# DSL-Lab/echoglad

Hardware: AMD Instinct MI355X
Metric: echo frames/sec through full GNN stack (224x224 default hier-graph); MAE parity (higher is better)
Workload: dtype f32; 1 GPU; configs[1] default.yml: 224x224 frame, 7 aux levels, num_gnn_layers=3, batch=8 per GPU, eval mode, node features [B*N,128] in HBM -> logits [B*N_valid,4] in HBM; workload_short=configs[1] default.yml: 224x224, 7 aux levels, L=3, batch 8/GPU, eval, nodes_per_frame=72020, directed_edges_per_frame=430200, global_batch=8, parallelism=dp1 (batch-sharded frames, no data-path collective), launch=hipGraph replay of the step's kernels

## Files before the change

echoglad_amd/build.py:

```python
from __future__ import annotations

import os
import shutil
import subprocess
import sys
from pathlib import Path

PKG = Path(__file__).resolve().parent
CSRC = PKG / "csrc"
LIBDIR = PKG / "lib"
LIBNAME = "libechoglad_hip.so"
SOURCES = ["graph.hip", "topo_tables.hip", "gcn_layer.hip", "gcn_layer_ps.hip", "conn.hip", "classifier.hip", "train.hip", "bn_act_tiles.hip", "cls_train.hip", "coord.hip", "coord_mlp.hip", "heatmap.hip", "pack.hip", "pool.hip", "adam.hip", "metrics.hip", "labels.hip", "frame_prep.hip", "frontend.hip", "frontend_train.hip", "embedder.hip"]
ARCH = "gfx950"


def hipcc() -> str:
    for cand in (os.environ.get("HIPCC"), shutil.which("hipcc"), "/opt/rocm/bin/hipcc"):
        if cand and os.path.exists(cand):
            return cand
    raise RuntimeError("hipcc not found; the HIP extension cannot be built")


def lib_path() -> Path:
    return LIBDIR / LIBNAME


def _stale(target: Path, deps) -> bool:
    if not target.exists():
        return True
    t = target.stat().st_mtime
    return any(Path(d).stat().st_mtime > t for d in deps)


def build(force: bool = False, verbose: bool = False, extra_flags=(), variant: str = "") -> Path:
    LIBDIR.mkdir(exist_ok=True)
    objdir = LIBDIR / ("obj" + ("_" + variant if variant else ""))
    objdir.mkdir(exist_ok=True)
    headers = list(CSRC.glob("*.h")) + [PKG.parent / "include" / "echoglad_hip.h"]
    cc = hipcc()
    flags = [f"--offload-arch={ARCH}", "-O3", "-fPIC", "-std=c++17", "-Wall", "-Wno-unused-function",
             "-mllvm", "-amdgpu-atomic-optimizer-strategy=None", *extra_flags]
    if verbose:
        flags.append("-Rpass-analysis=kernel-resource-usage")
    objs = []
    procs = []
    for src in SOURCES:
        s = CSRC / src
        if not s.exists():
            continue
        o = objdir / (s.stem + ".o")
        objs.append(o)
        if force or _stale(o, [s] + headers):
            cmd = [cc, *flags, "-c", str(s), "-o", str(o)]
            if verbose:
                print(" ".join(cmd), flush=True)
            procs.append((src, subprocess.Popen(cmd, stdout=subprocess.PIPE, stderr=subprocess.STDOUT, text=True)))
    for src, p in procs:
        out, _ = p.communicate()
        if verbose or p.returncode != 0:
            print(out, flush=True)
        if p.returncode != 0:
            raise RuntimeError(f"hipcc failed on {src}")
    target = lib_path() if not variant else LIBDIR / f"libechoglad_hip.{variant}.so"
    if force or _stale(target, objs):
        cmd = [cc, f"--offload-arch={ARCH}", "-shared", "-fPIC", "-o", str(target), *map(str, objs)]
        if verbose:
            print(" ".join(cmd), flush=True)
        subprocess.run(cmd, check=True)
    return target


if __name__ == "__main__":
    extra = [a for a in sys.argv[1:] if a.startswith("-D")]
    if "--" in sys.argv:
        extra += sys.argv[sys.argv.index("--") + 1:]
    var = [a.split("=", 1)[1] for a in sys.argv[1:] if a.startswith("--variant=")]
    p = build(force="--force" in sys.argv, verbose="--verbose" in sys.argv, extra_flags=extra,
              variant=var[0] if var else "")
    print(p)
```

echoglad_amd/csrc/common.h:

```cpp
#pragma once
#include <hip/hip_runtime.h>
#include <stdint.h>
#include <atomic>
#include <mutex>
#include <string>
#include <vector>

#include "../../include/echoglad_hip.h"

namespace eg {

constexpr int C = EG_CHANNELS;
constexpr int TILE = 64;
constexpr int LDA = C + 4;
constexpr int MAX_LEVELS = 14;
constexpr int MAX_SLOTS = 10;

int set_error(int code, const std::string& msg);
#define EG_HIP_TRY(expr)                                                                         \
    do {                                                                                         \
        hipError_t _e = (expr);                                                                  \
        if (_e != hipSuccess)                                                                    \
            return ::eg::set_error(EG_ERR_HIP, std::string(#expr) + ": " + hipGetErrorString(_e)); \
    } while (0)
// ... 75 lines not shown
    int r, c;
    if (is_main) {
        r = (int)(((unsigned long long)(unsigned)idx * T.magic) >> 40);
        c = idx - r * side;
    } else {
        const int lg = l + 1;
        r = idx >> lg;
        c = idx & (side - 1);
    }
    int deg = 0;
    nb.valid[1] = r > 0;            nb.id[1] = nb.valid[1] ? n - side : n;
    nb.valid[2] = r < side - 1;     nb.id[2] = nb.valid[2] ? n + side : n;
    nb.valid[3] = c > 0;            nb.id[3] = nb.valid[3] ? n - 1 : n;
    nb.valid[4] = c < side - 1;     nb.id[4] = nb.valid[4] ? n + 1 : n;
    deg += nb.valid[1] + nb.valid[2] + nb.valid[3] + nb.valid[4];
    if (is_main) {
        if (T.n_aux > 0 && r < 2 * T.ncrop && c < 2 * T.ncrop) {
            const int pl = T.n_levels - 2;
            nb.id[5] = T.base[pl] + (T.crop0 + (r >> 1)) * T.side[pl] + T.crop0 + (c >> 1);
            nb.valid[5] = 1; ++deg;
        }
        nb.count = 6;
    } else {
        if (l > 0) {
            nb.id[5] = T.base[l - 1] + (r >> 1) * T.side[l - 1] + (c >> 1);
            nb.valid[5] = 1; ++deg;
        }
        const int cl = l + 1;
        int cr = -1, cc = -1;
        if (cl < T.n_levels - 1) { cr = 2 * r; cc = 2 * c; }
        else if (r >= T.crop0 && r < T.crop0 + T.ncrop && c >= T.crop0 && c < T.crop0 + T.ncrop) {
            cr = 2 * (r - T.crop0); cc = 2 * (c - T.crop0);
        }
        if (cr >= 0) {
            const int cs = T.side[cl];
            const int b = T.base[cl] + cr * cs + cc;
            nb.id[6] = b;          nb.id[7] = b + 1;
            nb.id[8] = b + cs;     nb.id[9] = b + cs + 1;
            nb.valid[6] = nb.valid[7] = nb.valid[8] = nb.valid[9] = 1;
            deg += 4;
        }
        nb.count = 10;
    }
    nb.degree = deg;
}

enum GraphKind { GRAPH_TOPO = 1, GRAPH_CSR = 2 };

struct Knobs {
    int walk_mode;
    int stagger;
    int grid_cap;
    int layer_impl;
    int ps_grid;
    int ring_guard;
    int csr_tiles;
    int queue_self_reset;
};
Knobs read_knobs();
const Knobs& process_knobs();

constexpr int QUEUE_SLICE_INTS = 8 * 32;
constexpr int QUEUE_DONE_IDX = 1;
#ifdef EG_STAMP
constexpr int QUEUE_SLOTS = 1;
#else
constexpr int QUEUE_SLOTS = 64;
#endif
constexpr int QUEUE_TAIL_INTS = 64;
constexpr int EG_ERR_RING = -100;
inline int public_rc(int rc) { return rc == EG_ERR_RING ? EG_ERR_UNSUPPORTED : rc; }

}

struct eg_graph {
    int kind;
    int64_t n_nodes;
    eg::Topo topo;
    eg::Topo* topo_dev;
    eg::TileDesc* tiles_dev;
    eg::SegDesc* segs_dev;
    float* pats_dev;
    float* patsq_dev;
    int n_pats;
    int kid_rows;
    int hybrid;
    int n_conn;
    int conn_chunks;
    int* conn_table;
    mutable float* conn_scratch;
    mutable int conn_cap;
    mutable std::mutex conn_mutex;
    mutable std::vector<float*> conn_retired;
    int flat;
    int n_tiles;
    float* dis;
    int* rowptr;
    int* colidx;
    int64_t nnz;
    int* t_rows;
    int* t_rowptr;
    int* t_code;
    int* t_tgt;
    float* t_w;
    float* t_dis;
    int n_ctiles;
// ... 63 lines not shown
```

echoglad_amd/csrc/gcn_layer_ps.hip:

```cpp
#include <stdlib.h>

#include "seg_wide.h"
#include "train_common.h"

namespace eg {

constexpr int PS_THREADS = 512;
constexpr int PS_LDS_DIS = 4 * TILE * LDA + 16 + 64;
constexpr int PS_LDS_PAT = PS_LDS_DIS + 2 * TILE;

struct PsDims {
    int n_per_frame, batch, tiles_per_frame, relu, transpose_w, has_res;
    int kid_rows;
    int n_pats;
    float* agg_out;
    float* stats_partial;
    int static_walk;
    const float* res;
    const float* conn;
    int conn_stride, conn_agg, conn_scaled, n_conn;
    int self_reset;
    LowerSums lower;
};

// ... 22 lines not shown
#ifndef EG_PROBE_N
#define EG_PROBE_N 64
#endif
#define EG_PROBE(site) do { if ((site) == EG_PROBE_SITE) { int pa_ = lane, pb_ = lane; _Pragma("unroll") for (int i_ = 0; i_ < EG_PROBE_N / 2; ++i_) { \
    asm volatile("v_mov_b32 %0, %0" : "+v"(pa_)); asm volatile("v_mov_b32 %0, %0" : "+v"(pb_)); } asm volatile("" :: "v"(pa_), "v"(pb_)); } } while (0)
#else
#define EG_PROBE(site) do {} while (0)
#endif

__device__ inline int frame_of(int tile, int tiles_per_frame, int& hint) {
#ifdef EG_FRAME_HINT
    const unsigned t_in = (unsigned)(tile - hint * tiles_per_frame);
    if (t_in >= (unsigned)tiles_per_frame) hint = tile / tiles_per_frame;
    return hint;
#else
    (void)hint;
    return tile / tiles_per_frame;
#endif
}

__device__ inline float max_raw(float x, float y) {
    float r;
    asm("v_max_f32 %0, %1, %2" : "=v"(r) : "v"(x), "v"(y));
    return r;
}

__device__ inline int ps_claim_issue(int* __restrict__ counters, int group) {
    return atomicAdd(&counters[group * WALK_CTR_STRIDE], 1);
}
__device__ inline void ps_claim(int* __restrict__ counters, int group, int n_tiles, int* slot);
__device__ inline void ps_claim_commit(int* __restrict__ counters, int group, int n_tiles, int got, int* slot) {
    const int chunk = (n_tiles + WALK_GROUPS - 1) / WALK_GROUPS;
    const int lo = group * chunk;
    const int size = (n_tiles - lo) < chunk ? (n_tiles - lo) : chunk;
    if (got < size) *slot = lo + got;
    else ps_claim(counters, (group + 1) % WALK_GROUPS, n_tiles, slot);
}

__device__ inline void ps_claim(int* __restrict__ counters, int group, int n_tiles, int* slot) {
    const int chunk = (n_tiles + WALK_GROUPS - 1) / WALK_GROUPS;
    int t = -1;
    for (int k = 0; k < WALK_GROUPS && t < 0; ++k) {
        const int q = (group + k) % WALK_GROUPS;
        const int lo = q * chunk;
        const int size = (n_tiles - lo) < chunk ? (n_tiles - lo) : chunk;
        if (size <= 0) continue;
        const int got = atomicAdd(&counters[q * WALK_CTR_STRIDE], 1);
        if (got < size) t = lo + got;
    }
    *slot = t;
}


template <bool CLS, bool JK = false, int MODE = 0, bool DIAG = false, int FOLD = 0>
__global__ __launch_bounds__(PS_THREADS, 2) void k_gcn_layer_ps(const float* __restrict__ x, const float* __restrict__ W,
                                                                const float* __restrict__ scale, const float* __restrict__ shift,
                                                                float* __restrict__ out, const float* __restrict__ dis,
                                                                const Topo* __restrict__ T, const TileDesc* __restrict__ tiles,
                                                                const SegDesc* __restrict__ segs, const float* __restrict__ pats,
                                                                const float* __restrict__ patsq, const float* __restrict__ kin, float* __restrict__ kout,
                                                                const float* __restrict__ jk_in, float* __restrict__ jk_out,
                                                                int* __restrict__ counters, const PsDims a, const ClsArgs ca,
                                                                const int* __restrict__ rowptr, const int* __restrict__ colidx) {
    constexpr bool TRAIN = MODE == 1;
    constexpr bool RSEP = MODE >= 2;
    constexpr bool SUMS = MODE == 3;
    extern __shared__ __attribute__((aligned(16))) float smem[];
    float* s_a0 = smem;
    float* s_x0 = smem + 2 * TILE * LDA;
    int* s_tile = reinterpret_cast<int*>(smem + 4 * TILE * LDA);
    int* s_sync = s_tile + 8;
    int* s_cd = s_tile + 16;
    float* s_dis0 = smem + PS_LDS_DIS;
    float* s_pat = smem + PS_LDS_PAT;
    float* s_bn = s_pat + a.n_pats * PATQ;

    const int tid = threadIdx.x;
    const int lane_k = tid & 63;
    const int wave = wave_id();
    const bool consumer = wave < 4;
    const int n_tiles = a.tiles_per_frame * a.batch;
    const int group = xcc_id();

    if (tid == 256) {
        if (TRAIN && a.static_walk) {
            for (int i = 0; i < 3; ++i) s_tile[i] = ps_static_tile(i, n_tiles);
        } else {
            ps_claim(counters, group, n_tiles, &s_tile[0]);
            ps_claim(counters, group, n_tiles, &s_tile[1]);
            ps_claim(counters, group, n_tiles, &s_tile[2]);
        }
    }
    for (int i = tid; i < a.n_pats * PATQ; i += PS_THREADS) s_pat[i] = patsq[i];
    if (TRAIN) {
        for (int i = tid; i < 4 * TILE * LDA; i += PS_THREADS) smem[i] = 0.f;
    }
    static_assert(!FOLD || (CLS && !JK && MODE == 0), "FOLD is a form of the fused last layer without the running maximum");
    if (CLS) {
        if (FOLD) {
            if (tid < C) s_bn[tid] = ca.t1[tid];
        } else if (tid < C) {
            s_bn[tid] = scale ? scale[tid] : 1.0f;
            s_bn[C + tid] = shift ? shift[tid] : 0.0f;
            s_bn[2 * C + tid] = ca.s1[tid];
            s_bn[3 * C + tid] = ca.t1[tid];
        }
        if (tid == 0) *s_sync = 0;
    }
    __syncthreads();

    if (wave < 4) {
        constexpr bool RES_LATE = CLS;
        float wreg[64];
        load_w_slice(W, wave, lane_k, a.transpose_w, wreg);
        if (!FOLD && scale) {
            const float sv = scale[32 * wave + (lane_k & 31)];
#pragma unroll
            for (int t = 0; t < 64; ++t) wreg[t] *= sv;
        }
        f32x16 shv;
        if (!CLS) {
#pragma unroll
            for (int g = 0; g < 4; ++g) {
                const int ch0 = 32 * wave + 8 * g + 4 * (lane_k >> 5);
                const f32x4 q = shift ? *reinterpret_cast<const f32x4*>(shift + ch0) : f32x4{0.f, 0.f, 0.f, 0.f};
                shv[4 * g] = q.x; shv[4 * g + 1] = q.y; shv[4 * g + 2] = q.z; shv[4 * g + 3] = q.w;
            }
        }
        float wreg2[64];
        float w2a[8];
        f32x4 t2v, w3v;
        float b3v = 0.f;
        if (CLS) {
            load_w_slice(ca.w1, wave, lane_k, 0, wreg2);
            if (!FOLD) {
                const float sv = ca.s1[32 * wave + (lane_k & 31)];
#pragma unroll
                for (int t = 0; t < 64; ++t) wreg2[t] *= sv;
            }
            const f32x4* pw = reinterpret_cast<const f32x4*>(ca.w2 + (size_t)(wave * 16 + (lane_k & 15)) * 32 + 8 * (lane_k >> 4));
            const f32x4 q0 = pw[0], q1 = pw[1];
            w2a[0] = q0.x; w2a[1] = q0.y; w2a[2] = q0.z; w2a[3] = q0.w; w2a[4] = q1.x; w2a[5] = q1.y; w2a[6] = q1.z; w2a[7] = q1.w;
            {
                const float sv = ca.s2[wave * 16 + (lane_k & 15)];
#pragma unroll
                for (int t = 0; t < 8; ++t) w2a[t] *= sv;
            }
            const int o4 = wave * 16 + 4 * (lane_k >> 4);
            t2v = *reinterpret_cast<const f32x4*>(ca.t2 + o4);
            w3v = *reinterpret_cast<const f32x4*>(ca.w3 + o4);
            b3v = ca.b3[wave];
        }
        f32x16 csum, csq;
#pragma unroll
        for (int i = 0; i < 16; ++i) { csum[i] = 0.f; csq[i] = 0.f; }
        f32x4 lsc = {0.f, 0.f, 0.f, 0.f}, lsh = lsc;
        unsigned long long lseed = 0;
        if (SUMS) {
            lsc = *reinterpret_cast<const f32x4*>(a.lower.scale + 32 * wave + 4 * (lane_k & 7));
            lsh = *reinterpret_cast<const f32x4*>(a.lower.shift + 32 * wave + 4 * (lane_k & 7));
            lseed = a.lower.seed + epoch_now(a.lower.epoch);
        }
        __syncthreads();
        int frame_hint = 0;
        PSTAMP_INIT;
#ifdef EG_STAMP
        const unsigned long long clk0 = __builtin_amdgcn_s_memtime(), rt0 = __builtin_amdgcn_s_memrealtime();
#endif
        for (int k = 0;; ++k) {
            const int t_cur = __builtin_amdgcn_readfirstlane(s_tile[k & 7]);
            if (t_cur < 0) break;
            int lane = lane_k;
// ... 137 lines not shown
            auto read_segments = [&](int i0) {
#pragma unroll
                for (int e = 0; e < 4; ++e) {
                    if (JK) {
                        const int i = seg_cnt[i0 + e] > 0 ? i0 + e : 0;
                        const int cnt = seg_cnt[i0 + e] > 0 ? seg_cnt[i0 + e] : seg_cnt[0];
                        const int first = seg_cnt[i0 + e] > 0 ? seg_first[i0 + e] : seg_first[0];
                        const int u = u8 < cnt ? u8 : cnt - 1;
                        o[e] = *reinterpret_cast<const f32x4*>(s_x + (8 * i + u) * LDA + 32 * wave + c4);
                        node[e] = first + u;
                        ovoff[e] = u * (C * 4) + ocol;
                        osoff[e] = first * (C * 4);
                        jm[e] = *reinterpret_cast<const f32x4*>(jb + (size_t)node[e] * C);
                    } else {
                        const int last = seg_cnt[i0 + e] - 1;
                        const int u = u8 < last ? u8 : last;
                        o[e] = *reinterpret_cast<const f32x4*>(s_x + 8 * (i0 + e) * LDA + __mul24(u, LDA) + 32 * wave + c4);
                        ovoff[e] = u * (C * 4) + ocol;
                        osoff[e] = seg_first[i0 + e] * (C * 4);
                    }
                }
            };
            auto lower_sums = [&](int i0) {
#pragma unroll
                for (int e = 0; e < 4; ++e) {
                    const int node = seg_first[i0 + e] + u8;
                    const bool live = u8 < seg_cnt[i0 + e] && node < a.lower.row_hi;
                    f32x4 g = o[e];
                    if (a.lower.p > 0.f)
                        g *= keep_scale4(lseed, ((unsigned long long)frame * a.n_per_frame + node) * C + 32 * wave + c4, a.lower.p, a.lower.inv_keep);
                    const f32x4 zz = zr[i0 + e];
                    const f32x4 v = zz * lsc + lsh;
#pragma unroll
                    for (int u = 0; u < 4; ++u) {
                        const float ge = (live && (!a.lower.relu || v[u] > 0.f)) ? g[u] : 0.f;
                        ls1[u] += ge;
                        lt1[u] += ge * zz[u];
                    }
                }
            };
            auto store_segments = [&]() {
#pragma unroll
                for (int e = 0; e < 4; ++e) {
                    __builtin_amdgcn_raw_buffer_store_b128(__builtin_bit_cast(u32x4v, o[e]), orsrc, ovoff[e], osoff[e], 0);
                    if (JK) {
                        const f32x4 m = {fmaxf(jm[e].x, o[e].x), fmaxf(jm[e].y, o[e].y), fmaxf(jm[e].z, o[e].z), fmaxf(jm[e].w, o[e].w)};
                        *reinterpret_cast<f32x4*>(jo + (size_t)node[e] * C) = m;
                    }
                }
                store_data_guard(o);
            };
#ifndef EG_ABL_NO_MFMA
            auto between = [&](int c) {
                if (c < 2) { finish_group(acc0, 0, 2 * c); finish_group(acc0, 0, 2 * c + 1); }
                else if (!CLS && c == 2) read_segments(0);
                else if (!CLS) { store_segments(); if (SUMS) lower_sums(0); kout_half(0); }
                else if (c == 2) {
#pragma unroll
                    for (int g = 0; g < 4; ++g) res[0][g] = *reinterpret_cast<const f32x4*>(s_x + (32 + j) * LDA + 32 * wave + 4 * h + 8 * g);
                }
            };
#if defined(EG_EPI_MID)
            mfma_rowblock(s_a, 0, lane, wreg, acc0);
            asm volatile("" : "+v"(acc0));
            __builtin_amdgcn_sched_barrier(0);
            if (!CLS) {
#pragma unroll
                for (int g = 0; g < 4; ++g) finish_group(acc0, 0, g);
                read_segments(0); store_segments(); if (SUMS) lower_sums(0); kout_half(0);
            } else {
                between(0); between(1); between(2);
            }
            __builtin_amdgcn_sched_barrier(0);
            mfma_rowblock(s_a, 32, lane, wreg, acc1);
            asm volatile("" : "+v"(acc1));
            __builtin_amdgcn_sched_barrier(0);
#else
            if (!FOLD) {
                mfma_rowblock(s_a, 0, lane, wreg, acc0);
                mfma_rowblock_with(s_a, 32, lane, wreg, acc1, between);
            }
#endif
#else
            acc0[0] += wreg[0] + s_a[lane]; acc1[0] += wreg[63];
#pragma unroll
            for (int g = 0; g < 4; ++g) finish_group(acc0, 0, g);
            if (!CLS) { read_segments(0); store_segments(); if (SUMS) lower_sums(0); kout_half(0); }
#endif
            PSTAMP(0);
#ifdef EG_STAMP3
#pragma unroll
            for (int g = 0; g < EG_STAMP3; ++g) finish_group(acc1, 1, g);
            PSTAMP(3);
#pragma unroll
            for (int g = EG_STAMP3; g < 4; ++g) finish_group(acc1, 1, g);
#else
            if (!FOLD) {
#pragma unroll
                for (int g = 0; g < 4; ++g) finish_group(acc1, 1, g);
            }
#endif
            if (!CLS) {
                read_segments(4);
                store_segments();
                if (SUMS) {
                    lower_sums(4);
#pragma unroll
                    for (int m = 8; m < 64; m <<= 1) {
#pragma unroll
                        for (int u = 0; u < 4; ++u) { ls1[u] += __shfl_xor(ls1[u], m); lt1[u] += __shfl_xor(lt1[u], m); }
                    }
                    if (lane < 8) {
                        float* tp = a.lower.tile_partial + (size_t)t_cur * 2 * C + 32 * wave + 4 * lane;
                        *reinterpret_cast<f32x4*>(tp) = ls1;
                        *reinterpret_cast<f32x4*>(tp + C) = lt1;
                    }
                }
                kout_half(1);
            } else {
                PSTAMP(1);
                if (JK) {
                    const float* jb = jk_in + (size_t)frame * a.n_per_frame * C + 32 * wave + c4;
#pragma unroll
                    for (int i0 = 0; i0 < 8; i0 += 4) {
                        f32x4 jm[4];
                        int row[4];
#pragma unroll
                        for (int e = 0; e < 4; ++e) {
                            const int i = seg_cnt[i0 + e] > 0 ? i0 + e : 0;
                            const int cnt = seg_cnt[i0 + e] > 0 ? seg_cnt[i0 + e] : seg_cnt[0];
                            const int first = seg_cnt[i0 + e] > 0 ? seg_first[i0 + e] : seg_first[0];
// ... 315 lines not shown
                    }
                }
            }
            EG_PROBE(3);
            PSTAMP(2);
        };
        int dv_next = 0;
        {
            const int t0 = __builtin_amdgcn_readfirstlane(s_tile[0]);
            const int t1 = __builtin_amdgcn_readfirstlane(s_tile[1]);
            if (t0 >= 0) produce(t0, 0, lane_k, load_desc(t0, lane_k));
            if (t1 >= 0) dv_next = load_desc(t1, lane_k);
        }
        __syncthreads();
        for (int k = 0;; ++k) {
            const int t_cur = __builtin_amdgcn_readfirstlane(s_tile[k & 7]);
            if (t_cur < 0) break;
            const int t_next = __builtin_amdgcn_readfirstlane(s_tile[(k + 1) & 7]);
            const int t_nn = __builtin_amdgcn_readfirstlane(s_tile[(k + 2) & 7]);
            int lane = lane_k;
            asm volatile("" : "+v"(lane));
            const int dv_cur = dv_next;
            if (t_nn >= 0) dv_next = load_desc(t_nn, lane);
            int got = 0;
            const bool walk_static = TRAIN && a.static_walk;
            if (tid == 256 && !walk_static) got = ps_claim_issue(counters, group);
            PSTAMP(3);
            if (t_next >= 0) produce(t_next, (k + 1) & 1, lane, dv_cur);
            if (tid == 256) {
                if (walk_static) s_tile[(k + 3) & 7] = ps_static_tile(k + 3, n_tiles);
                else ps_claim_commit(counters, group, n_tiles, got, &s_tile[(k + 3) & 7]);
            }
            __syncthreads();
            PSTAMP(3);
        }
        if (TRAIN) {
            __syncthreads();
            __syncthreads();
        }
        PSTAMP_FLUSH(4);
#ifndef EG_STAMP
        if (tid == 256 && !(TRAIN && a.static_walk) && a.self_reset) {
            const int done = atomicAdd(&counters[QUEUE_DONE_IDX], 1);
            if (done == (int)gridDim.x - 1) {
#pragma unroll
                for (int q = 0; q < WALK_GROUPS; ++q) atomicExch(&counters[q * WALK_CTR_STRIDE], 0);
                atomicExch(&counters[QUEUE_DONE_IDX], 0);
            }
        }
#endif
    }
}

}

using namespace eg;

int eg_launch_conn_prepass(const eg_graph* g, int batch, const float* x, int slot, hipStream_t stream, const float** base);

int eg_launch_layer_ps(const eg_graph* g, int batch, const float* x, const float* W, const float* scale,
                       const float* shift, const float* residual, int relu, int transpose_w, float* out,
                       const float* kin, float* kout, const eg::ClsArgs* cls, hipStream_t stream, const float* jk_in, float* jk_out,
                       float* agg_out, float* stats_partial, int* grid_out, const eg::LowerSums* lower) {
    if (!g || g->kind != GRAPH_TOPO) return EG_ERR_UNSUPPORTED;
    if (lower && !(residual != nullptr && residual != x)) return set_error(EG_ERR_ARG, "the lower layer's sums go with the dX launch (a residual tensor of its own)");
    if (lower && (!lower->z || !lower->scale || !lower->shift || !lower->tile_partial || lower->row_hi < 1))
        return set_error(EG_ERR_ARG, "incomplete LowerSums");
    const bool train = stats_partial != nullptr;
    const bool rsep = residual != nullptr && residual != x;
    if (rsep && (train || kin || kout || cls || jk_in || jk_out)) return EG_ERR_UNSUPPORTED;
    if (agg_out && !train) return set_error(EG_ERR_ARG, "agg_out goes with stats_partial (train forward)");
    if (train && (kout || cls || jk_in || jk_out)) return set_error(EG_ERR_ARG, "the train forward writes no child sums (its activation pass does) and takes no heads or running maximum");
    const bool jk = jk_in != nullptr;
    if ((jk_out != nullptr) != (jk && !cls)) return set_error(EG_ERR_ARG, "jk_out goes with jk_in on a plain layer, the fused heads take jk_in alone");
    const bool chained = kin || kout || jk;
    if ((kin || kout) && g->kid_rows == 0) return EG_ERR_UNSUPPORTED;
    if (jk && g->kid_rows == 0 && !g->flat) return EG_ERR_UNSUPPORTED;
    if (cls && g->kid_rows == 0 && !g->flat) return EG_ERR_UNSUPPORTED;
    const bool diag = g->hybrid != 0;
    if (diag && jk) return EG_ERR_UNSUPPORTED;
    if (!chained && !cls && !train && !rsep && !diag &&
        (g->knobs.layer_impl < 0 ? (g->flat || g->kid_rows > 0) : g->knobs.layer_impl != 0) == false) return EG_ERR_UNSUPPORTED;
    PsDims a{};
    a.n_per_frame = (int)g->n_nodes; a.batch = batch; a.tiles_per_frame = g->n_tiles;
    a.relu = relu; a.transpose_w = transpose_w; a.has_res = residual != nullptr;
    a.kid_rows = g->kid_rows; a.n_pats = g->n_pats;
    a.agg_out = agg_out; a.stats_partial = stats_partial; a.static_walk = train ? 1 : 0;
    a.res = rsep ? residual : nullptr;
    if (lower) a.lower = *lower;
    const long long n_tiles = (long long)a.tiles_per_frame * batch;
    if (n_tiles <= 0) return EG_OK;
    const bool fold = cls && cls->fold;
    if (fold && (jk || relu || scale || shift)) return set_error(EG_ERR_ARG, "the folded heads take no running maximum, ReLU, scale or shift");
    const size_t lds = (size_t)(PS_LDS_PAT + g->n_pats * PATQ + (fold ? C : cls ? 4 * C : 0)) * sizeof(float);
    if (lds > 160 * 1024) return EG_ERR_UNSUPPORTED;
    {
        static std::atomic<bool> attr_set[64];
        int dev = 0;
        EG_HIP_TRY(hipGetDevice(&dev));
        if (dev < 0 || dev >= 64 || !attr_set[dev].load(std::memory_order_acquire)) {
            const void* kernels[] = {(const void*)k_gcn_layer_ps<false, false>, (const void*)k_gcn_layer_ps<true, false>,
                                     (const void*)k_gcn_layer_ps<false, true>, (const void*)k_gcn_layer_ps<true, true>,
                                     (const void*)k_gcn_layer_ps<false, false, 1>, (const void*)k_gcn_layer_ps<false, false, 2>,
                                     (const void*)k_gcn_layer_ps<false, false, 0, true>, (const void*)k_gcn_layer_ps<true, false, 0, true>,
                                     (const void*)k_gcn_layer_ps<false, false, 1, true>, (const void*)k_gcn_layer_ps<false, false, 2, true>,
                                     (const void*)k_gcn_layer_ps<false, false, 3>, (const void*)k_gcn_layer_ps<false, false, 3, true>,
                                     (const void*)k_gcn_layer_ps<true, false, 0, false, 1>, (const void*)k_gcn_layer_ps<true, false, 0, true, 1>,
                                     (const void*)k_gcn_layer_ps<true, false, 0, false, 2>, (const void*)k_gcn_layer_ps<true, false, 0, true, 2>};
            for (const void* f : kernels) EG_HIP_TRY(hipFuncSetAttribute(f, hipFuncAttributeMaxDynamicSharedMemorySize, 160 * 1024));
            if (dev >= 0 && dev < 64) attr_set[dev].store(true, std::memory_order_release);
        }
    }
    int* queue = nullptr;
    int slot = -1;
    {
        const int rc = g->acquire_queue_slice(stream, &queue, &slot);
        if (rc != EG_OK) return rc == EG_ERR_UNSUPPORTED ? EG_ERR_RING : rc;
    }
#ifdef EG_STAMP
    const bool self_reset = false;
    EG_HIP_TRY(hipMemsetAsync(queue, 0, sizeof(int) * QUEUE_SLICE_INTS, stream));
#else
    const bool self_reset = true;
    if (g->knobs.queue_self_reset == 0) {
        hipStreamCaptureStatus cs = hipStreamCaptureStatusNone;
        if (hipStreamIsCapturing(stream, &cs) != hipSuccess) { (void)hipGetLastError(); cs = hipStreamCaptureStatusNone; }
        if (cs == hipStreamCaptureStatusNone) EG_HIP_TRY(hipMemsetAsync(queue, 0, sizeof(int) * QUEUE_SLICE_INTS, stream));
    }
#endif
    a.self_reset = self_reset ? 1 : 0;
    if (g->n_conn > 0) {
        const float* slice = nullptr;
        const int rc = eg_launch_conn_prepass(g, batch, x, slot, stream, &slice);
        if (rc != EG_OK) return rc;
        a.conn = slice;
        a.conn_stride = (g->conn_chunks + 2 * g->n_conn) * C;
        a.conn_agg = g->conn_chunks * C;
        a.conn_scaled = (g->conn_chunks + g->n_conn) * C;
        a.n_conn = g->n_conn;
    }
    long long grid = n_tiles < 256 ? n_tiles : g->knobs.ps_grid;
    const ClsArgs none{};
    auto launch = [&](auto kernel) {
        hipLaunchKernelGGL(kernel, dim3((unsigned)grid), dim3(PS_THREADS), lds, stream, x, W, scale, shift, out, g->dis, g->topo_dev,
                           g->tiles_dev, g->segs_dev, g->pats_dev, g->patsq_dev, kin, kout, jk_in, jk_out, queue, a, cls ? *cls : none,
                           (const int*)g->rowptr, (const int*)g->colidx);
    };
    if (grid_out) *grid_out = (int)grid;
    eg::LaunchTimer timer(train ? EG_LAUNCH_PS_TRAIN_FWD : rsep ? EG_LAUNCH_PS_DX : cls ? EG_LAUNCH_PS_CLS : EG_LAUNCH_PS_PLAIN, stream);
    if (diag) {
        if (train) launch(k_gcn_layer_ps<false, false, 1, true>);
        else if (rsep && lower) launch(k_gcn_layer_ps<false, false, 3, true>);
        else if (rsep) launch(k_gcn_layer_ps<false, false, 2, true>);
        else if (fold) { if (residual) launch(k_gcn_layer_ps<true, false, 0, true, 1>); else launch(k_gcn_layer_ps<true, false, 0, true, 2>); }
        else if (cls) launch(k_gcn_layer_ps<true, false, 0, true>);
        else launch(k_gcn_layer_ps<false, false, 0, true>);
    } else if (train) launch(k_gcn_layer_ps<false, false, 1>);
    else if (rsep && lower) launch(k_gcn_layer_ps<false, false, 3>);
    else if (rsep) launch(k_gcn_layer_ps<false, false, 2>);
    else if (fold) { if (residual) launch(k_gcn_layer_ps<true, false, 0, false, 1>); else launch(k_gcn_layer_ps<true, false, 0, false, 2>); }
    else if (cls) { if (jk) launch(k_gcn_layer_ps<true, true>); else launch(k_gcn_layer_ps<true, false>); }
    else { if (jk) launch(k_gcn_layer_ps<false, true>); else launch(k_gcn_layer_ps<false, false>); }
    g->commit_queue_slice(slot, stream);
    g->ps_launches.fetch_add(1u, std::memory_order_relaxed);
    g->layer_launches.fetch_add(1u, std::memory_order_relaxed);
    EG_HIP_TRY(hipGetLastError());
    return EG_OK;
}
```

echoglad_amd/csrc/graph.hip:

```cpp
#include <hipcub/hipcub.hpp>

#include <cmath>
#include <memory>
#include <vector>

#include "topo_tables.h"
#include <cstring>

namespace eg {

static thread_local std::string g_last_error;

int set_error(int code, const std::string& msg) {
    g_last_error = msg;
    return code;
}

#define EG_NO_STREAM_YET ((void*)(intptr_t)-1)

static int env_int(const char* name, int dflt) {
    const char* v = getenv(name);
    return v && *v ? atoi(v) : dflt;
}

Knobs read_knobs() {
    Knobs k;
    k.layer_impl = env_int("EG_LAYER_IMPL", -1);
    k.csr_tiles = env_int("EG_CSR_TILES", 2);
#ifndef EG_WALK_MODE
#define EG_WALK_MODE 0
#endif
#ifndef EG_STAGGER
#define EG_STAGGER 0
#endif
#ifndef EG_GRID
#define EG_GRID 512
#endif
#ifndef EG_PS_GRID
#define EG_PS_GRID 256
#endif
#ifndef EG_RING_GUARD
#define EG_RING_GUARD 1
#endif
#ifndef EG_QUEUE_SELF_RESET
#define EG_QUEUE_SELF_RESET 1
#endif
    k.walk_mode = EG_WALK_MODE;
    k.stagger = EG_STAGGER;
    k.grid_cap = EG_GRID;
    k.ps_grid = EG_PS_GRID;
    k.ring_guard = EG_RING_GUARD;
    k.queue_self_reset = EG_QUEUE_SELF_RESET != 0;
    if (k.ps_grid < 8) k.ps_grid = 8;
    if (k.ps_grid > 2048) k.ps_grid = 2048;
    if (k.grid_cap < 8) k.grid_cap = 8;
    if (k.grid_cap > 2048) k.grid_cap = 2048;
    return k;
}

const Knobs& process_knobs() {
    static const Knobs k = read_knobs();
    return k;
}

constexpr size_t QUEUE_RING_BYTES = sizeof(int) * ((size_t)QUEUE_SLOTS * QUEUE_SLICE_INTS + QUEUE_TAIL_INTS);

}

int eg_graph::acquire_queue_slice(hipStream_t stream, int** slice, int* slot) const {
    const unsigned s = launch_seq.fetch_add(1u, std::memory_order_relaxed) % (unsigned)eg::QUEUE_SLOTS;
    {
        void* none = EG_NO_STREAM_YET;
        only_stream.compare_exchange_strong(none, (void*)stream, std::memory_order_acq_rel);
        any_launch.store(1, std::memory_order_release);
    }
    hipStreamCaptureStatus cap = hipStreamCaptureStatusNone;
    if (hipStreamIsCapturing(stream, &cap) != hipSuccess) { (void)hipGetLastError(); cap = hipStreamCaptureStatusNone; }
    if (any_launch.load(std::memory_order_acquire) && !multi_stream.load(std::memory_order_acquire) &&
        only_stream.load(std::memory_order_acquire) != (void*)stream) {
        hipStream_t old = (hipStream_t)only_stream.load(std::memory_order_acquire);
        if (cap == hipStreamCaptureStatusNone) {
// ... 460 lines not shown
```

echoglad_amd/csrc/tile.h:

```cpp
#pragma once
#include "common.h"

namespace eg {

typedef float f32x16 __attribute__((ext_vector_type(16)));
typedef float f32x4 __attribute__((ext_vector_type(4)));
typedef float f32x2 __attribute__((ext_vector_type(2)));

enum Agg { AGG_NONE = 0, AGG_CSR = 1, AGG_STENCIL = 2, AGG_CSRT = 3 };

__device__ inline int wave_id() { return __builtin_amdgcn_readfirstlane((int)(threadIdx.x >> 6)); }

__device__ inline f32x2 load_row2(const float* __restrict__ base, int row, int lane) {
    const unsigned off = (unsigned)row * (unsigned)C + 2u * (unsigned)lane;
    return *reinterpret_cast<const f32x2*>(base + off);
}

__device__ inline f32x2 agg_stencil(const Topo* __restrict__ Tp, const float* __restrict__ xf, const float* __restrict__ dis,
                                    int n, int lane) {
    Nbrs nb;
    neighbours(*Tp, n, nb);
    float w[MAX_SLOTS];
#pragma unroll
    for (int s = 0; s < MAX_SLOTS; ++s) {
// ... 395 lines not shown
    const int j = lane & 31, h = lane >> 5;
    const f32x4* ap = reinterpret_cast<const f32x4*>(s_a + (row0 + j) * LDA + 64 * h);
    f32x4 a0[4], a1[4];
#pragma unroll
    for (int t = 0; t < 4; ++t) a0[t] = ap[t];
#pragma unroll
    for (int t = 0; t < 4; ++t) a1[t] = ap[4 + t];
    __builtin_amdgcn_sched_barrier(0);
    mfma_chunk<true>(a0, wreg, 0, acc);
#pragma unroll
    for (int t = 0; t < 4; ++t) a0[t] = ap[8 + t];
    __builtin_amdgcn_sched_barrier(0);
    mfma_chunk<true>(a1, wreg, 4, acc);
#pragma unroll
    for (int t = 0; t < 4; ++t) a1[t] = ap[12 + t];
    __builtin_amdgcn_sched_barrier(0);
    mfma_chunk<true>(a0, wreg, 8, acc);
    __builtin_amdgcn_sched_barrier(0);
    mfma_chunk<true>(a1, wreg, 12, acc);
}

#ifdef EG_CLUMP
#define EG_CLUMP_FENCE do { asm volatile("" : "+v"(acc)); __builtin_amdgcn_sched_barrier(0); } while (0)
#else
#define EG_CLUMP_FENCE do {} while (0)
#endif
template <typename F>
__device__ inline void mfma_rowblock_with(const float* s_a, int row0, int lane, const float (&wreg)[64], f32x16& acc, F between) {
    const int j = lane & 31, h = lane >> 5;
    const f32x4* ap = reinterpret_cast<const f32x4*>(s_a + (row0 + j) * LDA + 64 * h);
    f32x4 a0[4], a1[4];
#pragma unroll
    for (int t = 0; t < 4; ++t) a0[t] = ap[t];
#pragma unroll
    for (int t = 0; t < 4; ++t) a1[t] = ap[4 + t];
    __builtin_amdgcn_sched_barrier(0);
    mfma_chunk(a0, wreg, 0, acc);
    EG_CLUMP_FENCE; between(0); EG_CLUMP_FENCE;
#pragma unroll
    for (int t = 0; t < 4; ++t) a0[t] = ap[8 + t];
    __builtin_amdgcn_sched_barrier(0);
    mfma_chunk(a1, wreg, 4, acc);
    EG_CLUMP_FENCE; between(1); EG_CLUMP_FENCE;
#pragma unroll
    for (int t = 0; t < 4; ++t) a1[t] = ap[12 + t];
    __builtin_amdgcn_sched_barrier(0);
    mfma_chunk(a0, wreg, 8, acc);
    EG_CLUMP_FENCE; between(2); EG_CLUMP_FENCE;
    __builtin_amdgcn_sched_barrier(0);
    mfma_chunk(a1, wreg, 12, acc);
    EG_CLUMP_FENCE; between(3); EG_CLUMP_FENCE;
}

typedef float f32x4v __attribute__((ext_vector_type(4)));

__device__ inline int koff16(int kq) { return ((kq & 1) << 6) | ((kq & 2) << 4); }

__device__ inline void load_w_slice16(const float* __restrict__ W, int wave, int lane, int transpose, float (&wreg)[32]) {
    const int i = lane & 15, k0 = koff16(lane >> 4);
    if (!transpose) {
        const f32x4* p = reinterpret_cast<const f32x4*>(W + (size_t)(16 * wave + i) * C + k0);
#pragma unroll
        for (int t = 0; t < 8; ++t) {
            const f32x4 q = p[t];
            wreg[4 * t + 0] = q.x; wreg[4 * t + 1] = q.y; wreg[4 * t + 2] = q.z; wreg[4 * t + 3] = q.w;
        }
    } else {
        const float* p = W + (size_t)k0 * C + 16 * wave + i;
#pragma unroll
        for (int s = 0; s < 32; ++s) wreg[s] = p[(size_t)s * C];
    }
}

template <bool PREFETCH = true>
__device__ inline void mfma16_pair(const float* s_a, int row0, int lane, const float (&wreg)[32], f32x4v& accA, f32x4v& accB) {
    const int j = lane & 15, k0 = koff16(lane >> 4);
    const f32x4* pa = reinterpret_cast<const f32x4*>(s_a + (row0 + j) * LDA + k0);
    const f32x4* pb = reinterpret_cast<const f32x4*>(s_a + (row0 + 16 + j) * LDA + k0);
    f32x4 fa[4], fb[4];
#pragma unroll
    for (int t = 0; t < 4; ++t) { fa[t] = pa[t]; fb[t] = pb[t]; }
#pragma unroll
    for (int c = 0; c < 2; ++c) {
        f32x4 ga[4], gb[4];
        if (PREFETCH && c == 0) {
#pragma unroll
            for (int t = 0; t < 4; ++t) { ga[t] = pa[4 + t]; gb[t] = pb[4 + t]; }
        }
        __builtin_amdgcn_sched_barrier(0);
#pragma unroll
        for (int t = 0; t < 4; ++t) {
            const int w0 = 16 * c + 4 * t;
            accA = __builtin_amdgcn_mfma_f32_16x16x4f32(wreg[w0 + 0], fa[t].x, accA, 0, 0, 0);
            accB = __builtin_amdgcn_mfma_f32_16x16x4f32(wreg[w0 + 0], fb[t].x, accB, 0, 0, 0);
            accA = __builtin_amdgcn_mfma_f32_16x16x4f32(wreg[w0 + 1], fa[t].y, accA, 0, 0, 0);
            accB = __builtin_amdgcn_mfma_f32_16x16x4f32(wreg[w0 + 1], fb[t].y, accB, 0, 0, 0);
            accA = __builtin_amdgcn_mfma_f32_16x16x4f32(wreg[w0 + 2], fa[t].z, accA, 0, 0, 0);
            accB = __builtin_amdgcn_mfma_f32_16x16x4f32(wreg[w0 + 2], fb[t].z, accB, 0, 0, 0);
            accA = __builtin_amdgcn_mfma_f32_16x16x4f32(wreg[w0 + 3], fa[t].w, accA, 0, 0, 0);
            accB = __builtin_amdgcn_mfma_f32_16x16x4f32(wreg[w0 + 3], fb[t].w, accB, 0, 0, 0);
        }
        if (c == 0) {
            if (!PREFETCH) {
#pragma unroll
                for (int t = 0; t < 4; ++t) { ga[t] = pa[4 + t]; gb[t] = pb[4 + t]; }
            }
// ... 92 lines not shown
```

Before: 10290 frames/s.

## Add bf16x6 split-precision MFMA path for plain eval GCN layer

```diff
diff --git a/echoglad_amd/build.py b/echoglad_amd/build.py
--- a/echoglad_amd/build.py
+++ b/echoglad_amd/build.py
@@ -10,8 +10,37 @@
 CSRC = PKG / "csrc"
 LIBDIR = PKG / "lib"
 LIBNAME = "libechoglad_hip.so"
-SOURCES = ["graph.hip", "topo_tables.hip", "gcn_layer.hip", "gcn_layer_ps.hip", "conn.hip", "classifier.hip", "train.hip", "bn_act_tiles.hip", "cls_train.hip", "coord.hip", "coord_mlp.hip", "heatmap.hip", "pack.hip", "pool.hip", "adam.hip", "metrics.hip", "labels.hip", "frame_prep.hip", "frontend.hip", "frontend_train.hip", "embedder.hip"]
+SOURCES = ["graph.hip", "topo_tables.hip", "gcn_layer.hip", "gcn_layer_ps.hip", "gcn_layer_ps_split.hip", "conn.hip", "classifier.hip", "train.hip", "bn_act_tiles.hip", "cls_train.hip", "coord.hip", "coord_mlp.hip", "heatmap.hip", "pack.hip", "pool.hip", "adam.hip", "metrics.hip", "labels.hip", "frame_prep.hip", "frontend.hip", "frontend_train.hip", "embedder.hip"]
 ARCH = "gfx950"
+FILE_FLAGS = {"gcn_layer_ps_split.hip": ["-Xclang", "-target-feature", "-Xclang", "-packed-fp32-ops"]}
+FILE_DEPS = {"gcn_layer_ps_split.hip": ["gcn_layer_ps.hip"]}
+NO_PACKED_FP32 = ("gcn_layer_ps_split.hip",)
+LLVM_BIN = Path("/opt/rocm/lib/llvm/bin")
+
+
+def device_disassembly(binary: Path) -> str:
+    import re
+    import tempfile
+    with tempfile.TemporaryDirectory(prefix="eg_build_") as tmp:
+        fat = Path(tmp) / "fatbin"
+        subprocess.run(["objcopy", "-O", "binary", "--only-section=.hip_fatbin", str(binary), str(fat)], check=True)
+        blob = fat.read_bytes()
+        starts = [m.start() for m in re.finditer(re.escape(b"__CLANG_OFFLOAD_BUNDLE__"), blob)]
+        text = []
+        for i, a in enumerate(starts):
+            piece, out = Path(tmp) / f"bundle{i}", Path(tmp) / f"{ARCH}_{i}.co"
+            piece.write_bytes(blob[a:starts[i + 1] if i + 1 < len(starts) else len(blob)])
+            r = subprocess.run([str(LLVM_BIN / "clang-offload-bundler"), "--unbundle", "--type=o", f"--input={piece}",
+                                f"--targets=hipv4-amdgcn-amd-amdhsa--{ARCH}", f"--output={out}"], capture_output=True)
+            if r.returncode == 0 and out.exists() and out.stat().st_size > 0:
+                text.append(subprocess.run([str(LLVM_BIN / "llvm-objdump"), "-d", str(out)], check=True, capture_output=True, text=True).stdout)
+    return "\n".join(text)
+
+
+def packed_fp32_census(binary: Path):
+    import re
+    text = device_disassembly(binary)
+    return len(re.findall(r"\bv_mfma_f32_32x32x16_bf16\b", text)), len(re.findall(r"\bv_pk_\w+_f32\b", text))
 
 
 def hipcc() -> str:
@@ -50,8 +79,8 @@
             continue
         o = objdir / (s.stem + ".o")
         objs.append(o)
-        if force or _stale(o, [s] + headers):
-            cmd = [cc, *flags, "-c", str(s), "-o", str(o)]
+        if force or _stale(o, [s] + [CSRC / d for d in FILE_DEPS.get(src, [])] + headers):
+            cmd = [cc, *flags, *FILE_FLAGS.get(src, []), "-c", str(s), "-o", str(o)]
             if verbose:
                 print(" ".join(cmd), flush=True)
             procs.append((src, subprocess.Popen(cmd, stdout=subprocess.PIPE, stderr=subprocess.STDOUT, text=True)))
@@ -61,6 +90,13 @@
             print(out, flush=True)
         if p.returncode != 0:
             raise RuntimeError(f"hipcc failed on {src}")
+        if src in NO_PACKED_FP32:
+            o = objdir / (Path(src).stem + ".o")
+            n_mfma, n_packed = packed_fp32_census(o)
+            if n_mfma == 0 or n_packed != 0:
+                o.unlink()
+                raise RuntimeError(f"{src}: {n_mfma} bf16 MFMAs and {n_packed} packed fp32 instructions in the device code; "
+                                   "expected some and none (packed fp32 instructions beside bf16 MFMAs return wrong results)")
     target = lib_path() if not variant else LIBDIR / f"libechoglad_hip.{variant}.so"
     if force or _stale(target, objs):
         cmd = [cc, f"--offload-arch={ARCH}", "-shared", "-fPIC", "-o", str(target), *map(str, objs)]
diff --git a/echoglad_amd/csrc/common.h b/echoglad_amd/csrc/common.h
--- a/echoglad_amd/csrc/common.h
+++ b/echoglad_amd/csrc/common.h
@@ -151,6 +151,7 @@
     int stagger;
     int grid_cap;
     int layer_impl;
+    int layer_split;
     int ps_grid;
     int ring_guard;
     int csr_tiles;
diff --git a/echoglad_amd/csrc/gcn_layer_ps.hip b/echoglad_amd/csrc/gcn_layer_ps.hip
--- a/echoglad_amd/csrc/gcn_layer_ps.hip
+++ b/echoglad_amd/csrc/gcn_layer_ps.hip
@@ -98,7 +98,7 @@
 }
 
 
-template <bool CLS, bool JK = false, int MODE = 0, bool DIAG = false, int FOLD = 0>
+template <bool CLS, bool JK = false, int MODE = 0, bool DIAG = false, int FOLD = 0, bool SPLIT = false>
 __global__ __launch_bounds__(PS_THREADS, 2) void k_gcn_layer_ps(const float* __restrict__ x, const float* __restrict__ W,
                                                                 const float* __restrict__ scale, const float* __restrict__ shift,
                                                                 float* __restrict__ out, const float* __restrict__ dis,
@@ -142,6 +142,7 @@
         for (int i = tid; i < 4 * TILE * LDA; i += PS_THREADS) smem[i] = 0.f;
     }
     static_assert(!FOLD || (CLS && !JK && MODE == 0), "FOLD is a form of the fused last layer without the running maximum");
+    static_assert(!SPLIT || (!CLS && !JK && MODE == 0), "SPLIT is a form of the plain eval layer");
     if (CLS) {
         if (FOLD) {
             if (tid < C) s_bn[tid] = ca.t1[tid];
@@ -156,7 +157,7 @@
     __syncthreads();
 
     if (wave < 4) {
-        constexpr bool RES_LATE = CLS;
+        constexpr bool RES_LATE = CLS || SPLIT;
         float wreg[64];
         load_w_slice(W, wave, lane_k, a.transpose_w, wreg);
         if (!FOLD && scale) {
@@ -164,6 +165,8 @@
 #pragma unroll
             for (int t = 0; t < 64; ++t) wreg[t] *= sv;
         }
+        WPieces wp;
+        if constexpr (SPLIT) split_w_slice(wreg, wp);
         f32x16 shv;
         if (!CLS) {
 #pragma unroll
@@ -407,9 +410,15 @@
             };
 #ifndef EG_ABL_NO_MFMA
             auto between = [&](int c) {
-                if (c < 2) { finish_group(acc0, 0, 2 * c); finish_group(acc0, 0, 2 * c + 1); }
+                if (c < 2) {
+                    finish_group(acc0, 0, 2 * c); finish_group(acc0, 0, 2 * c + 1);
+                    if (SPLIT && c == 1) {
+#pragma unroll
+                        for (int g = 0; g < 4; ++g) res[0][g] = *reinterpret_cast<const f32x4*>(s_x + (32 + j) * LDA + 32 * wave + 4 * h + 8 * g);
+                    }
+                }
                 else if (!CLS && c == 2) read_segments(0);
-                else if (!CLS) { store_segments(); if (SUMS) lower_sums(0); kout_half(0); }
+                else if (!CLS) { store_segments(); if (SUMS) lower_sums(0); if (!SPLIT) kout_half(0); }
                 else if (c == 2) {
 #pragma unroll
                     for (int g = 0; g < 4; ++g) res[0][g] = *reinterpret_cast<const f32x4*>(s_x + (32 + j) * LDA + 32 * wave + 4 * h + 8 * g);
@@ -431,7 +440,11 @@
             asm volatile("" : "+v"(acc1));
             __builtin_amdgcn_sched_barrier(0);
 #else
-            if (!FOLD) {
+            if constexpr (SPLIT) {
+                mfma_rowblock_bf16x6(s_a, 0, lane, wp, acc0);
+                mfma_rowblock_bf16x6_with(s_a, 32, lane, wp, acc1, between);
+                kout_half(0);
+            } else if (!FOLD) {
                 mfma_rowblock(s_a, 0, lane, wreg, acc0);
                 mfma_rowblock_with(s_a, 32, lane, wreg, acc1, between);
             }
@@ -853,8 +866,17 @@
     }
 }
 
+using PsKernelFn = decltype(&k_gcn_layer_ps<false>);
+PsKernelFn ps_split_kernel(bool diag);
+#ifdef EG_PS_SPLIT_TU
+PsKernelFn ps_split_kernel(bool diag) {
+    return diag ? k_gcn_layer_ps<false, false, 0, true, 0, true> : k_gcn_layer_ps<false, false, 0, false, 0, true>;
 }
-
+#endif
+
+}
+
+#ifndef EG_PS_SPLIT_TU
 using namespace eg;
 
 int eg_launch_conn_prepass(const eg_graph* g, int batch, const float* x, int slot, hipStream_t stream, const float** base);
@@ -907,7 +929,8 @@
                                      (const void*)k_gcn_layer_ps<false, false, 1, true>, (const void*)k_gcn_layer_ps<false, false, 2, true>,
                                      (const void*)k_gcn_layer_ps<false, false, 3>, (const void*)k_gcn_layer_ps<false, false, 3, true>,
                                      (const void*)k_gcn_layer_ps<true, false, 0, false, 1>, (const void*)k_gcn_layer_ps<true, false, 0, true, 1>,
-                                     (const void*)k_gcn_layer_ps<true, false, 0, false, 2>, (const void*)k_gcn_layer_ps<true, false, 0, true, 2>};
+                                     (const void*)k_gcn_layer_ps<true, false, 0, false, 2>, (const void*)k_gcn_layer_ps<true, false, 0, true, 2>,
+                                     (const void*)ps_split_kernel(false), (const void*)ps_split_kernel(true)};
             for (const void* f : kernels) EG_HIP_TRY(hipFuncSetAttribute(f, hipFuncAttributeMaxDynamicSharedMemorySize, 160 * 1024));
             if (dev >= 0 && dev < 64) attr_set[dev].store(true, std::memory_order_release);
         }
@@ -949,22 +972,25 @@
     };
     if (grid_out) *grid_out = (int)grid;
     eg::LaunchTimer timer(train ? EG_LAUNCH_PS_TRAIN_FWD : rsep ? EG_LAUNCH_PS_DX : cls ? EG_LAUNCH_PS_CLS : EG_LAUNCH_PS_PLAIN, stream);
+    const bool split = g->knobs.layer_split != 0;
     if (diag) {
         if (train) launch(k_gcn_layer_ps<false, false, 1, true>);
         else if (rsep && lower) launch(k_gcn_layer_ps<false, false, 3, true>);
         else if (rsep) launch(k_gcn_layer_ps<false, false, 2, true>);
         else if (fold) { if (residual) launch(k_gcn_layer_ps<true, false, 0, true, 1>); else launch(k_gcn_layer_ps<true, false, 0, true, 2>); }
         else if (cls) launch(k_gcn_layer_ps<true, false, 0, true>);
+        else if (split) launch(ps_split_kernel(true));
         else launch(k_gcn_layer_ps<false, false, 0, true>);
     } else if (train) launch(k_gcn_layer_ps<false, false, 1>);
     else if (rsep && lower) launch(k_gcn_layer_ps<false, false, 3>);
     else if (rsep) launch(k_gcn_layer_ps<false, false, 2>);
     else if (fold) { if (residual) launch(k_gcn_layer_ps<true, false, 0, false, 1>); else launch(k_gcn_layer_ps<true, false, 0, false, 2>); }
     else if (cls) { if (jk) launch(k_gcn_layer_ps<true, true>); else launch(k_gcn_layer_ps<true, false>); }
-    else { if (jk) launch(k_gcn_layer_ps<false, true>); else launch(k_gcn_layer_ps<false, false>); }
+    else { if (jk) launch(k_gcn_layer_ps<false, true>); else if (split) launch(ps_split_kernel(false)); else launch(k_gcn_layer_ps<false, false>); }
     g->commit_queue_slice(slot, stream);
     g->ps_launches.fetch_add(1u, std::memory_order_relaxed);
     g->layer_launches.fetch_add(1u, std::memory_order_relaxed);
     EG_HIP_TRY(hipGetLastError());
     return EG_OK;
 }
+#endif
diff --git a/echoglad_amd/csrc/gcn_layer_ps_split.hip b/echoglad_amd/csrc/gcn_layer_ps_split.hip
--- /dev/null
+++ b/echoglad_amd/csrc/gcn_layer_ps_split.hip
@@ -0,0 +1,2 @@
+#define EG_PS_SPLIT_TU
+#include "gcn_layer_ps.hip"
diff --git a/echoglad_amd/csrc/graph.hip b/echoglad_amd/csrc/graph.hip
--- a/echoglad_amd/csrc/graph.hip
+++ b/echoglad_amd/csrc/graph.hip
@@ -27,6 +27,7 @@
     Knobs k;
     k.layer_impl = env_int("EG_LAYER_IMPL", -1);
     k.csr_tiles = env_int("EG_CSR_TILES", 2);
+    k.layer_split = env_int("EG_LAYER_SPLIT", 1);
 #ifndef EG_WALK_MODE
 #define EG_WALK_MODE 0
 #endif
diff --git a/echoglad_amd/csrc/tile.h b/echoglad_amd/csrc/tile.h
--- a/echoglad_amd/csrc/tile.h
+++ b/echoglad_amd/csrc/tile.h
@@ -471,6 +471,125 @@
     EG_CLUMP_FENCE; between(3); EG_CLUMP_FENCE;
 }
 
+__host__ __device__ inline float split3_top16(float v) {
+    unsigned u;
+    __builtin_memcpy(&u, &v, 4);
+    u &= 0xFFFF0000u;
+    float r;
+    __builtin_memcpy(&r, &u, 4);
+    return r;
+}
+__host__ __device__ inline void split3(float a, float& hi, float& mid, float& lo) {
+    hi = split3_top16(a);
+    const float r = a - hi;
+    mid = split3_top16(r);
+    lo = split3_top16(r - mid);
+}
+
+typedef __bf16 bf16x8 __attribute__((ext_vector_type(8)));
+typedef unsigned u32x4 __attribute__((ext_vector_type(4)));
+
+__device__ inline unsigned pack_top16(float e0, float e1) {
+    return __builtin_amdgcn_perm(__float_as_uint(e1), __float_as_uint(e0), 0x07060302u);
+}
+struct Pieces { bf16x8 hi, mid, lo; };
+
+__device__ inline Pieces split3_x8(const f32x4& q0, const f32x4& q1) {
+    float hi[8], mid[8], lo[8];
+#pragma unroll
+    for (int e = 0; e < 4; ++e) { split3(q0[e], hi[e], mid[e], lo[e]); split3(q1[e], hi[4 + e], mid[4 + e], lo[4 + e]); }
+    u32x4 ph, pm, pl;
+#pragma unroll
+    for (int e = 0; e < 4; ++e) {
+        ph[e] = pack_top16(hi[2 * e], hi[2 * e + 1]);
+        pm[e] = pack_top16(mid[2 * e], mid[2 * e + 1]);
+        pl[e] = pack_top16(lo[2 * e], lo[2 * e + 1]);
+    }
+    return Pieces{__builtin_bit_cast(bf16x8, ph), __builtin_bit_cast(bf16x8, pm), __builtin_bit_cast(bf16x8, pl)};
+}
+
+struct WPieces { bf16x8 hi[8], mid[8], lo[8]; };
+__device__ inline void split_w_slice(const float (&wreg)[64], WPieces& wp) {
+#pragma unroll
+    for (int t = 0; t < 8; ++t) {
+        const Pieces p = split3_x8(f32x4{wreg[8 * t], wreg[8 * t + 1], wreg[8 * t + 2], wreg[8 * t + 3]},
+                                   f32x4{wreg[8 * t + 4], wreg[8 * t + 5], wreg[8 * t + 6], wreg[8 * t + 7]});
+        wp.hi[t] = p.hi; wp.mid[t] = p.mid; wp.lo[t] = p.lo;
+    }
+}
+
+__device__ inline void mfma_operand_guard(const f32x16& acc) {
+    __builtin_amdgcn_sched_barrier(0);
+    const int seen = __builtin_amdgcn_readfirstlane(__float_as_int(acc[0]));
+    asm volatile("" :: "s"(seen));
+#ifndef EG_SPLIT_GUARD_NOPS
+#define EG_SPLIT_GUARD_NOPS 1
+#endif
+#pragma unroll
+    for (int i = 0; i < EG_SPLIT_GUARD_NOPS; ++i) asm volatile("s_nop 15" ::: "memory");
+    __builtin_amdgcn_sched_barrier(0);
+}
+__device__ inline void keep_pieces(const Pieces& p) {
+    const u32x4 a = __builtin_bit_cast(u32x4, p.hi), b = __builtin_bit_cast(u32x4, p.mid), c = __builtin_bit_cast(u32x4, p.lo);
+    asm volatile("" :: "v"(a.x), "v"(a.y), "v"(a.z), "v"(a.w), "v"(b.x), "v"(b.y), "v"(b.z), "v"(b.w), "v"(c.x), "v"(c.y), "v"(c.z), "v"(c.w));
+    __builtin_amdgcn_sched_barrier(0);
+}
+
+template <int PART>
+__device__ inline void mfma_step_bf16x6(const WPieces& wp, int t, const Pieces& ap, f32x16& acc) {
+    if (PART == 0) {
+        acc = __builtin_amdgcn_mfma_f32_32x32x16_bf16(wp.lo[t], ap.hi, acc, 0, 0, 0);
+    } else {
+        acc = __builtin_amdgcn_mfma_f32_32x32x16_bf16(wp.hi[t], ap.lo, acc, 0, 0, 0);
+        acc = __builtin_amdgcn_mfma_f32_32x32x16_bf16(wp.mid[t], ap.mid, acc, 0, 0, 0);
+        acc = __builtin_amdgcn_mfma_f32_32x32x16_bf16(wp.mid[t], ap.hi, acc, 0, 0, 0);
+        acc = __builtin_amdgcn_mfma_f32_32x32x16_bf16(wp.hi[t], ap.mid, acc, 0, 0, 0);
+        acc = __builtin_amdgcn_mfma_f32_32x32x16_bf16(wp.hi[t], ap.hi, acc, 0, 0, 0);
+    }
+}
+
+template <typename F>
+__device__ inline void mfma_rowblock_bf16x6_with(const float* s_a, int row0, int lane, const WPieces& wp, f32x16& acc, F between) {
+    const int j = lane & 31, h = lane >> 5;
+    const f32x4* ap = reinterpret_cast<const f32x4*>(s_a + (row0 + j) * LDA + 64 * h);
+    f32x4 raw[2][2];
+    Pieces set[2];
+    raw[0][0] = ap[0]; raw[0][1] = ap[1];
+    raw[1][0] = ap[2]; raw[1][1] = ap[3];
+    set[0] = split3_x8(raw[0][0], raw[0][1]);
+    __builtin_amdgcn_sched_barrier(0);
+#pragma unroll
+    for (int t = 0; t < 8; ++t) {
+        const Pieces& cur = set[t & 1];
+        keep_pieces(cur);
+        mfma_step_bf16x6<0>(wp, t, cur, acc);
+        if (t >= 1) {
+            mfma_operand_guard(acc);
+            keep_pieces(set[(t + 1) & 1]);
+        }
+        __builtin_amdgcn_sched_barrier(0);
+        if (t < 7) set[(t + 1) & 1] = split3_x8(raw[(t + 1) & 1][0], raw[(t + 1) & 1][1]);
+        if (t < 6) { raw[t & 1][0] = ap[2 * (t + 2)]; raw[t & 1][1] = ap[2 * (t + 2) + 1]; }
+        mfma_step_bf16x6<1>(wp, t, cur, acc);
+        if (t & 1) between(t >> 1);
+        if (t < 7) {
+#pragma unroll
+            for (int q = 0; q < 5; ++q) {
+                __builtin_amdgcn_sched_group_barrier(0x008, 1, 0);
+                __builtin_amdgcn_sched_group_barrier(0x002, 9, 0);
+            }
+        }
+        __builtin_amdgcn_sched_barrier(0);
+    }
+    mfma_operand_guard(acc);
+    keep_pieces(set[0]);
+    keep_pieces(set[1]);
+}
+
+__device__ inline void mfma_rowblock_bf16x6(const float* s_a, int row0, int lane, const WPieces& wp, f32x16& acc) {
+    mfma_rowblock_bf16x6_with(s_a, row0, lane, wp, acc, [](int) {});
+}
+
 typedef float f32x4v __attribute__((ext_vector_type(4)));
 
 __device__ inline int koff16(int kq) { return ((kq & 1) << 6) | ((kq & 2) << 4); }
```

Result: faster. 10920 frames/s (median of 6 runs) (+6.1%).
